# ParBLiSS/FastANI

Measured on AMD Instinct MI355X. Metric: ANI pairs/sec, many-to-many NxN ~5 Mbp genomes, higher is better.
Workload: dtype u32

## Files before the change

fastani_amd/csrc/engine_core.hip:

```cpp
#include "host/engine.hpp"
#include "kernels/scan.hpp"
#include "kernels/synth.hpp"

namespace anih {

thread_local std::string g_err;

int fail(int code, const char *fmt, ...)
{
  char buf[1024];
  va_list ap; va_start(ap, fmt); vsnprintf(buf, sizeof buf, fmt, ap); va_end(ap);
  g_err = buf;
  return code;
}

DevicePool g_pools[64];

int zero_counters(ani_ctx *c)
{
  HIP_TRY(hipMemsetAsync(c->dCounters.p, 0, kCounterWords * 8, c->stream));
  return ANI_OK;
}
int zero_cursors(ani_ctx *c, int pool)
{
// ... 133 lines not shown
  if (const char *ev = getenv("ANI_TEST_L2_OVERLAP")) c->l2Overlap = strcmp(ev, "0") != 0;
  if (const char *ev = getenv("ANI_TEST_L1_HIT_LIMIT")) { const long long v = atoll(ev);
    if (v >= 1) c->l1HitLimit = std::min<uint64_t>((uint64_t)v, 0x7ffffff0ull); }
  if (const char *ev = getenv("ANI_TEST_CAND_POOL_MIN")) { const long long v = atoll(ev); if (v >= 1) c->candPoolMin = (uint64_t)v; }
  if (const char *ev = getenv("ANI_TEST_L1_BIG_GROUP_HITS")) { const long long v = atoll(ev); if (v >= 1) c->l1BigGroupHits = (uint64_t)v; }
  if (const char *ev = getenv("ANI_TEST_L1_BIG_GROUP_FRAGS")) { const long long v = atoll(ev); if (v >= 1) c->l1BigGroupFrags = (uint64_t)v; }
  if (const char *ev = getenv("ANI_MAX_RESIDENT_CHUNKS")) { const long long v = atoll(ev);
    if (v >= 0) c->maxResidentChunks = (int32_t)std::min<long long>(v, 1 << 20); }
  if (const char *ev = getenv("ANI_STREAM_CHUNK_MINIMIZERS")) { const long long v = atoll(ev); if (v >= 1) c->streamChunkMinimizers = (uint64_t)v; }
  for (int i = 0; i < 2; i++) { HIP_TRY(hipEventCreateWithFlags(&c->evSimA[i], hipEventDisableTiming));
    HIP_TRY(hipEventCreateWithFlags(&c->evSetDone[i], hipEventDisableTiming)); HIP_TRY(hipEventCreateWithFlags(&c->evIndex[i], hipEventDisableTiming)); }
  int rc = c->dCounters.ensure(kCounterWords * 8);
  if (rc != ANI_OK) { delete c; return rc; }
  *out = c;
  return ANI_OK;
}

void ani_shutdown(ani_ctx *c)
{
  if (!c) return;
  (void)hipSetDevice(c->device);
  DevBuf *bufs[] = {&c->dCounters, &c->seqPacked, &c->seqAscii, &c->contigOff, &c->contigLen, &c->contigMode, &c->sortTmp, &c->unitStart, &c->unitAux,
      &c->tiles, &c->tileInfo, &c->tileMeta, &c->tileCnt,
                    &c->tileDrop, &c->tileOff, &c->poolHash, &c->poolWpos, &c->scanTmpA, &c->scanTmpB, &c->scanTmpC, &c->scanTmpD, &c->frags, &c->fragOff,
                        &c->fragS,
                    &c->fragGenome, &c->fragQSeq, &c->qPool, &c->l1FragDesc, &c->probeFirst, &c->probeCnt, &c->l1MidList, &c->l1SmallList, &c->l1BigList,
                        &c->l1BigHitsA, &c->l1BigHitsB, &c->l1BigV, &c->l1BigTbl, &c->l1BigHash, &c->candFrag, &c->candSeq, &c->candStart, &c->candEnd,
                        &c->fragCandOff, &c->fragCandCnt,
                    &c->fragCandCntClamped, &c->fragHits, &c->fragOrdOff, &c->fragOrder, &c->fragOrderTmp, &c->ocFrag, &c->ocSeq, &c->ocStart, &c->ocEnd,
                        &c->l2Scratch, &c->l2Ranges[0], &c->l2CodeCount[0], &c->l2CodeOff[0], &c->l2Codes[0], &c->l2SlowFlag[0], &c->l2ClassList[0],
                        &c->l2Order[0], &c->l2LenHist[0],
                    &c->l2Ranges[1], &c->l2CodeCount[1], &c->l2CodeOff[1], &c->l2Codes[1], &c->l2SlowFlag[1], &c->l2ClassList[1], &c->l2Order[1],
                        &c->l2LenHist[1], &c->l2SlowList, &c->l2Best,
                    &c->l2First, &c->l2Last, &c->refStart, &c->idBits, &c->keepFlags, &c->keepOff, &c->mapOut, &c->bins, &c->queryFragments, &c->rows};
  for (DevBuf *b : bufs) b->release();
  for (hipEvent_t e : c->timerEvents) if (e) (void)hipEventDestroy(e);
  for (int i = 0; i < 2; i++) { if (c->evSimA[i]) (void)hipEventDestroy(c->evSimA[i]); if (c->evSetDone[i]) (void)hipEventDestroy(c->evSetDone[i]);
    if (c->evIndex[i]) (void)hipEventDestroy(c->evIndex[i]); }
  if (c->stream2) (void)hipStreamDestroy(c->stream2);
  for (int i = 0; i < 5; i++) if (c->pinned[i]) (void)hipHostFree(c->pinned[i]);
  if (c->stream) (void)hipStreamDestroy(c->stream);
  delete c;
  cur_pool().trim();
}

int ani_device_copy(ani_ctx *c, void *dst, const void *src, size_t bytes)
{
  if (!c || (bytes && (!dst || !src))) return fail(ANI_ERR_ARG, "null argument");
  HIP_TRY(hipSetDevice(c->device));
  if (bytes) { HIP_TRY(hipMemcpyAsync(dst, src, bytes, hipMemcpyDefault, c->stream)); HIP_TRY(hipStreamSynchronize(c->stream)); }
  return ANI_OK;
}

int ani_device_alloc(ani_ctx *c, size_t bytes, void **out)
{
  if (!c || !out) return fail(ANI_ERR_ARG, "null argument");
  HIP_TRY(hipSetDevice(c->device));
  HIP_TRY(pool_malloc(out, bytes ? bytes : 1));
  return ANI_OK;
}

int ani_device_memory(ani_ctx *c, size_t *freeBytes, size_t *totalBytes)
{
  if (!c) return fail(ANI_ERR_ARG, "null argument");
  HIP_TRY(hipSetDevice(c->device));
  size_t f = 0, t = 0;
  HIP_TRY(hipMemGetInfo(&f, &t));
// ... 81 lines not shown
```

fastani_amd/csrc/engine_map.hip:

```cpp
#include <atomic>
#include <thread>
#include "host/engine.hpp"
#include "kernels/l1.hpp"
#include "kernels/l2.hpp"
#include "kernels/reduce.hpp"
#include "kernels/cluster.hpp"
#include "kernels/tree.hpp"
#include "kernels/nj.hpp"
#include "kernels/single.hpp"
#include "kernels/sigdist.hpp"
#include "kernels/sigstrip.hpp"
#include "kernels/signeigh.hpp"
#include "kernels/sigscreen.hpp"
#include "kernels/sigcontain.hpp"
#include "kernels/sigcluster.hpp"
#include "kernels/siggraph.hpp"

namespace anih {
using namespace ani;

void launch_l2_codes(unsigned grid, hipStream_t s, const L2FastArgs &fa);
void launch_l2_sim_a(unsigned grid, hipStream_t s, const L2FastArgs &fa, const int32_t *list, const unsigned int *listCount);
void launch_l2_sim_b(unsigned grid, hipStream_t s, const L2FastArgs &fa, const int32_t *list, const unsigned int *listCount);
static_assert(kL1FilterMinHits == 300 && kL1HitCapMax == 4080, "defaults of ani_ctx::l1FilterMin / l1LdsMax (host/engine.hpp)");
// ... 315 lines not shown
    if (nSlowTotal) {
      size_t lanes = (std::min<size_t>(nSlowTotal, (size_t)1 << 17) + kTPB - 1) / kTPB * kTPB;
      const size_t wordsPerLane = (size_t)maxS + 1;
      while (lanes > kTPB && lanes * wordsPerLane * 4 > ((size_t)2 << 30)) lanes = (lanes / 2 + kTPB - 1) / kTPB * kTPB;
      TRY(ctx->l2Scratch.ensure(lanes * wordsPerLane * 4));
      L2Args sa = a; sa.scratch = ctx->l2Scratch.as<uint32_t>(); sa.laneStride = lanes;
      StageTimer tk(ctx, &ctx->counters.msL2Slow, 1);
      for (size_t base = 0; base < nSlowTotal; base += lanes)
        hipLaunchKernelGGL(k_l2, dim3((unsigned)(lanes / kTPB)), dim3(kTPB), 0, ctx->stream, sa, (const int32_t *)ctx->l2SlowList.as<int32_t>(),
            (int32_t)nSlowTotal, (int32_t)base);
      HIP_TRY(hipGetLastError());
    }
    ctx->counters.l2SlowCandidates += nSlowTotal; ctx->counters.l2FastCandidates += nCand - nSlowTotal;
    FinishArgs fa;
    fa.nCand = (int32_t)nCand; fa.candFrag = a.candFrag; fa.candSeq = a.candSeq; fa.best = a.outBest; fa.firstPos = a.outFirst; fa.lastPos = a.outLast;
    fa.fragS = a.fragS; fa.idLUT = set->dIdLUT; fa.minShared = set->dMinShared; fa.lutMaxS = set->dLutMaxS;
    fa.refStart = ctx->refStart.as<int32_t>(); fa.idBits = ctx->idBits.as<uint32_t>();
    hipLaunchKernelGGL(k_finish_candidates, dim3(grid_for(nCand)), dim3(256), 0, ctx->stream, fa);
    HIP_TRY(hipGetLastError());
  }
  TRY(read_counters(ctx, host));
  ctx->counters.l2WindowEntries += host[CNT_ENTRIES] + host[CNT_ENTRIES_B]; ctx->counters.l2Steps += host[CNT_STEPS] + host[CNT_STEPS_B];
  ctx->counters.l2QueryHashes += host[CNT_SUMQ] + host[CNT_SUMQ_B];
  ctx->counters.l2WindowEntriesB += host[CNT_ENTRIES_B]; ctx->counters.l2QueryHashesB += host[CNT_SUMQ_B];
  ctx->counters.l2SlowLimit += host[CNT_REASON + 1]; ctx->counters.l2SlowDup += host[CNT_REASON + 2]; ctx->counters.l2SlowOverflow += host[CNT_REASON + 3];
  return ANI_OK;
}

int reduce_stage(ani_ctx *ctx, ani_sketch *set, IndexChunk *sk, const FragSet &fs, int32_t nCand, int32_t nQuery, bool compact = false)
{
  if (nQuery == 0 || sk->nGenomes == 0) return ANI_OK;
  const size_t binsPerQuery = sk->totalBins;
  const size_t nBins = binsPerQuery * (size_t)nQuery;
  TRY(ctx->bins.ensure((nBins ? nBins : 1) * 4));
  const size_t nPairsAll = (size_t)nQuery * (size_t)(compact ? sk->nGenomes : set->nGenomes);
  TRY(ctx->rows.ensure((nPairsAll ? nPairsAll : 1) * 8));
  hipError_t e1;
  {
  StageTimer tm(ctx, &ctx->counters.msReduce);
  e1 = hipMemsetAsync(ctx->bins.p, 0, (nBins ? nBins : 1) * 4, ctx->stream);
  if (nCand) {
    OneWayArgs a;
    a.nCand = nCand; a.candFrag = ctx->ocFrag.as<int32_t>(); a.candSeq = ctx->ocSeq.as<int32_t>(); a.refStart = ctx->refStart.as<int32_t>();
    a.idBits = ctx->idBits.as<uint32_t>(); a.fragGenome = fs.fragGenome; a.genomeBase = fs.genomeBase; a.contigGenome = sk->contigGenome;
    a.contigBinBase = sk->contigBinBase; a.binWidth = set->params.fragLen - 20; a.bins = ctx->bins.as<uint32_t>(); a.binsPerQuery = binsPerQuery;
    hipLaunchKernelGGL(k_oneway_bins, dim3(grid_for((size_t)nCand)), dim3(256), 0, ctx->stream, a);
  }
  PairArgs pa;
  pa.nQuery = nQuery; pa.nRefGenomes = sk->nGenomes; pa.bins = ctx->bins.as<uint32_t>(); pa.binsPerQuery = binsPerQuery;
  pa.genomeBinStart = sk->genomeBinStart; pa.pairCount = ctx->rows.as<uint32_t>(); pa.pairIdentity = ctx->rows.as<uint32_t>() + nPairsAll;
  pa.outStride = compact ? sk->nGenomes : set->nGenomes; pa.outCol0 = compact ? 0 : sk->g0;
  const size_t nPairs = (size_t)nQuery * (size_t)sk->nGenomes;
  hipLaunchKernelGGL(k_pair_reduce, dim3((unsigned)((nPairs + 3) / 4)), dim3(256), 0, ctx->stream, pa);
  }
  HIP_TRY(e1); HIP_TRY(hipGetLastError());
  return ANI_OK;
}

int collect_rows(ani_ctx *ctx, ani_sketch *set, const FragSet &fs, int32_t nQuery, int32_t firstQueryId, RowBuf *rows, const IndexChunk *block = nullptr,
    const int32_t *queryIds = nullptr)
{
  const int32_t nCols = block ? block->nGenomes : set->nGenomes, col0 = (block ? block->g0 : 0) + set->refIdBase;
  const size_t nPairs = (size_t)nQuery * (size_t)nCols;
  if (nPairs == 0) return ANI_OK;
  uint32_t *dense = nullptr;
  TRY(pinned_buffer(ctx, 1, nPairs * 8 + 8, (void **)&dense));
  HIP_TRY(hipMemcpyAsync(dense, ctx->rows.p, nPairs * 8, hipMemcpyDeviceToHost, ctx->stream));
  HIP_TRY(hipStreamSynchronize(ctx->stream));
  std::vector<size_t> qOff((size_t)nQuery + 1, 0);
  parallel_for((size_t)nQuery, (uint64_t)nPairs * 8, [&](size_t qi) {
    const uint32_t *cnt = dense + qi * (size_t)nCols;
    size_t c = 0;
    for (int32_t g = 0; g < nCols; g++) c += cnt[g] != 0;
    qOff[qi + 1] = c;
  });
  for (int32_t qi = 0; qi < nQuery; qi++) qOff[qi + 1] += qOff[qi];
  const size_t m = qOff[nQuery];
  ani_cgi_t *out0 = rows->grow(m);
  if (!out0) return fail(ANI_ERR_NOMEM, "host allocation of %zu result rows failed", m);
  rows->n += m;
  parallel_for((size_t)nQuery, (uint64_t)nPairs * 8, [&](size_t qi) {
    const uint32_t *cnt = dense + qi * (size_t)nCols, *idb = cnt + nPairs;
    ani_cgi_t *out = out0 + qOff[qi];
    for (int32_t g = 0; g < nCols; g++) {
      if (!cnt[g]) continue;
      ani_cgi_t r; r.refGenomeId = col0 + g; r.qryGenomeId = firstQueryId + (queryIds ? queryIds[qi] : (int32_t)qi); r.countSeq = (int32_t)cnt[g];
      r.totalQueryFragments = fs.genomeFragments[qi];
      memcpy(&r.identity, &idb[g], 4);
// ... 1747 lines not shown
```

fastani_amd/csrc/engine_sketch.hip:

```cpp
#include "host/engine.hpp"
#include "kernels/reduce.hpp"
#include "kernels/sketch.hpp"

namespace anih {
using namespace ani;

int check_params(const ani_params_t *p)
{
  if (!p) return fail(ANI_ERR_ARG, "null parameters");
  if (p->kmerSize < 1 || p->kmerSize > 16) return fail(ANI_ERR_ARG, "kmerSize must be in 1..16 (hash_t is 32 bit, parseCmdArgs.hpp:142)");
  if (p->windowSize < 1 || p->windowSize > ani::kTile - ani::kTPB) return fail(ANI_ERR_LIMIT, "windowSize %d outside 1..%d", p->windowSize,
      ani::kTile - ani::kTPB);
  if (p->fragLen < 1 || p->fragLen <= 20) return fail(ANI_ERR_ARG, "fragLen must exceed 20 (bin width is fragLen-20, computeCoreIdentity.hpp:194)");
  return ANI_OK;
}

int frag_tables(ani_ctx *ctx, const ani_params_t &p, const DeviceBatch &db, FragSet *qr, std::vector<uint32_t> *fragStartOut, const FragArrays &fa, bool alloc,
                FragArrays *owned)
{
  const int k = p.kmerSize, w = p.windowSize, L = p.fragLen;
  std::vector<uint32_t> &fragStart = *fragStartOut;
  fragStart.assign((size_t)db.nContigs + 1, 0);
  std::vector<int32_t> cGenome((size_t)db.nContigs + 1, 0), cQBase((size_t)db.nContigs + 1, 0);
  qr->genomeFragments.assign(db.nGenomes, 0);
// ... 123 lines not shown
    TRY(ctx->poolHash.ensure(cap * 4)); TRY(ctx->poolWpos.ensure(cap * 4));
    if (fused && (!*fused->qPool || attempt > 0)) {
      if (*fused->qPool) { pool_free(*fused->qPool); *fused->qPool = nullptr; }
      HIP_TRY(pool_malloc((void **)fused->qPool, (qcap ? qcap : 1) * 4));
    }
    TRY(zero_counters(ctx));
    {
      StageTimer tm(ctx, &ctx->counters.msSketch);
      if (!fused)
        hipLaunchKernelGGL(k_sketch_tiles, dim3((unsigned)nT), dim3(kTPB), 0, ctx->stream, db.dPacked, db.dAscii, db.dContigOff,
                           db.dContigLen, db.dContigMode, ctx->tiles.as<TileDesc>(), k, w, ctx->poolHash.as<uint32_t>(),
                           ctx->poolWpos.as<int32_t>(), stripe_cap(cap), cur_ptr(ctx, POOL_REF), ctx->tileMeta.as<TileMeta>());
      else
        hipLaunchKernelGGL(k_sketch_fused, dim3((unsigned)nT), dim3(kTPB), 0, ctx->stream, db.dPacked, db.dAscii, db.dContigOff, db.dContigLen, db.dContigMode,
                           ctx->tiles.as<TileDesc>(), ctx->tileInfo.as<FusedInfo>(), k, w, L, ctx->poolHash.as<uint32_t>(), ctx->poolWpos.as<int32_t>(),
                               stripe_cap(cap),
                           cur_ptr(ctx, POOL_REF), ctx->tileMeta.as<TileMeta>(), *fused->qPool, stripe_cap(qcap), cur_ptr(ctx,
                               POOL_Q), fused->arr->fragOff, fused->arr->fragS,
                           (int *)cnt_ptr(ctx, CNT_MAXS));
    }
    HIP_TRY(hipGetLastError());
    TRY(read_counters(ctx, host));
    const bool refFits = ctx->poolMaxStripe[POOL_REF] <= stripe_cap(cap), qFits = !fused || ctx->poolMaxStripe[POOL_Q] <= stripe_cap(qcap);
    if (refFits && qFits) break;
    if (attempt > 2) return fail(ANI_ERR_INTERNAL, "minimizer pool did not converge");
    if (!refFits) cap = grown_cap(ctx->poolMaxStripe[POOL_REF]);
    if (!qFits) qcap = grown_cap(ctx->poolMaxStripe[POOL_Q]);
  }
  if (fused) {
    const int maxS = (int)(uint32_t)host[CNT_MAXS];
    if (maxS >= 0x7fffffff) return fail(ANI_ERR_LIMIT, "a query fragment produced more than %d minimizers", kFragHashCap);
    const uint64_t nHashes = ctx->poolUsed[POOL_Q];
    ctx->counters.querySketchHashes += nHashes;
    uint32_t *packed = nullptr;
    TRY(compact_fragment_pool(ctx, *fused->qPool, fused->arr->fragOff, fused->arr->fragS, nF, nHashes, &packed));
    pool_free(*fused->qPool); *fused->qPool = packed;
    fused->fs->maxS = maxS; fused->fs->nHashes = nHashes; fused->fs->poolSize = nHashes; fused->fs->qPool = *fused->qPool;
  }
  StageTimer tm(ctx, &ctx->counters.msSketch);
  hipLaunchKernelGGL(k_sketch_tile_counts, dim3(grid_for(nT)), dim3(256), 0, ctx->stream, ctx->tiles.as<TileDesc>(),
                     ctx->tileMeta.as<TileMeta>(), (int)nT, ctx->tileCnt.as<int32_t>(), ctx->tileDrop.as<uint8_t>());
  uint64_t total = 0;
  TRY(device_scan(ctx, ctx->tileCnt.as<int32_t>(), ctx->tileOff.as<uint32_t>(), (uint32_t)nT, &total));
  if (total >= 0x7ffffff0ull) return fail(ANI_ERR_LIMIT, "reference batch yields >= 2^31 minimizers; split the reference list");
  if (total == 0) return ANI_OK;
  uint32_t *rec = nullptr;
  HIP_TRY(pool_malloc((void **)&rec, total * 12));
  hipLaunchKernelGGL(k_sketch_gather, dim3((unsigned)nT), dim3(kTPB), 0, ctx->stream, ctx->tiles.as<TileDesc>(), ctx->tileMeta.as<TileMeta>(),
                     ctx->tileDrop.as<uint8_t>(), ctx->tileOff.as<uint32_t>(), ctx->poolHash.as<uint32_t>(), ctx->poolWpos.as<int32_t>(),
                     seqIdBase, rec);
  hipError_t e = hipGetLastError();
  if (e == hipSuccess) e = hipStreamSynchronize(ctx->stream);
  if (e != hipSuccess) { pool_free(rec); HIP_TRY(e); }
  *dRecords = rec; *nOut = (size_t)total;
  return ANI_OK;
}

int fragment_stage(ani_ctx *ctx, const ani_params_t &p, const DeviceBatch &db, FragSet *qr)
{
  if (ctx->timerPending.size() > 4096) flush_timers(ctx);
  const int k = p.kmerSize, w = p.windowSize, L = p.fragLen;
  {
    uint64_t nF = 0;
    for (int32_t c = 0; c < db.nContigs; c++) { const int32_t len = db.contigLen[c]; if (!(len < w || len < k || len < L)) nF += (uint64_t)(len / L); }
    TRY(ctx->fragOff.ensure((nF + 1) * 4)); TRY(ctx->fragS.ensure((nF + 1) * 4)); TRY(ctx->fragGenome.ensure((nF + 1) * 4));
    TRY(ctx->fragQSeq.ensure((nF + 1) * 4));
  }
  FragArrays fa; fa.fragOff = ctx->fragOff.as<uint32_t>(); fa.fragS = ctx->fragS.as<int32_t>(); fa.fragGenome = ctx->fragGenome.as<int32_t>();
  fa.fragQSeq = ctx->fragQSeq.as<int32_t>();
  std::vector<uint32_t> fragStart;
// ... 32 lines not shown
  qr->qPool = ctx->qPool.as<uint32_t>();
  return ANI_OK;
}

void fragset_release(ani_fragset *f)
{
  void *tables[] = {f->arr.fragOff, f->arr.fragS, f->arr.fragGenome, f->arr.fragQSeq};
  if (!f->borrowed || f->ownTables) for (void *q : tables) if (q) pool_free(q);
  if (!f->borrowed && f->qPool) pool_free(f->qPool);
  delete f;
}
void fragset_finish(ani_fragset *f)
{
  f->genomeFragStart.assign(f->fs.genomeFragments.size() + 1, 0);
  for (size_t g = 0; g < f->fs.genomeFragments.size(); g++) f->genomeFragStart[g + 1] = f->genomeFragStart[g] + f->fs.genomeFragments[g];
}
int keep_fragment_arrays(ani_ctx *ctx, ani_fragset *f)
{
  const size_t nF = (size_t)f->fs.nFrag;
  if (!nF) return ANI_OK;
  hipError_t e = pool_malloc((void **)&f->arr.fragOff, nF * 4); if (e == hipSuccess) e = pool_malloc((void **)&f->arr.fragS, nF * 4);
  if (e == hipSuccess) e = pool_malloc((void **)&f->arr.fragGenome, nF * 4); if (e == hipSuccess) e = pool_malloc((void **)&f->arr.fragQSeq, nF * 4);
  if (e == hipSuccess) e = hipMemcpyAsync(f->arr.fragOff, f->fs.fragOff, nF * 4, hipMemcpyDeviceToDevice, ctx->stream);
  if (e == hipSuccess) e = hipMemcpyAsync(f->arr.fragS, f->fs.fragS, nF * 4, hipMemcpyDeviceToDevice, ctx->stream);
  if (e == hipSuccess) e = hipMemcpyAsync(f->arr.fragGenome, f->fs.fragGenome, nF * 4, hipMemcpyDeviceToDevice, ctx->stream);
  if (e == hipSuccess) e = hipMemcpyAsync(f->arr.fragQSeq, f->fs.fragQSeq, nF * 4, hipMemcpyDeviceToDevice, ctx->stream);
  if (e != hipSuccess) return fail(e == hipErrorOutOfMemory ? ANI_ERR_NOMEM : ANI_ERR_DEVICE, "keeping the fragment sketches failed: %s", hipGetErrorString(e));
  TRY(compact_fragment_pool(ctx, f->fs.qPool, f->arr.fragOff, f->arr.fragS, nF, f->fs.nHashes, &f->qPool));
  f->fs.fragOff = f->arr.fragOff; f->fs.fragS = f->arr.fragS; f->fs.fragGenome = f->arr.fragGenome; f->fs.fragQSeq = f->arr.fragQSeq;
  f->fs.qPool = f->qPool; f->fs.poolSize = f->fs.nHashes;
  return ANI_OK;
}

int records_of_batch(ani_ctx *ctx, const ani_params_t *p, const ani_seq_batch_t *refs, int32_t seqIdBase, void **devRecords, size_t *n, ani_fragset *keep)
{
  std::vector<RecordPart> parts;
  auto cleanup = [&]() { for (auto &q : parts) if (q.rec) pool_free(q.rec); };
  size_t total = 0;
  int32_t g0 = 0;
  while (g0 < refs->nGenomes) {
    int32_t g1 = g0; uint64_t bases = 0;
    while (g1 < refs->nGenomes && (g1 == g0 || keep || bases < (1ull << 30))) {
      for (int32_t c = refs->genomeContigStart[g1]; c < refs->genomeContigStart[g1 + 1]; c++) bases += (uint64_t)refs->contigLen[c];
      g1++;
    }
    DeviceBatch db;
    int rc = upload_batch(ctx, refs, g0, g1, &db);
    RecordPart pt; pt.g0 = g0; pt.g1 = g1;
    if (rc == ANI_OK) {
      if (keep && fusable(p)) {
        FusedOut fo{&keep->fs, &keep->arr, &keep->qPool};
        rc = sketch_records(ctx, p, db, seqIdBase + refs->genomeContigStart[g0], &pt.rec, &pt.n, &fo);
      } else {
        rc = sketch_records(ctx, p, db, seqIdBase + refs->genomeContigStart[g0], &pt.rec, &pt.n);
        if (rc == ANI_OK && keep) {
          rc = fragment_stage(ctx, *p, db, &keep->fs);
          if (rc == ANI_OK) rc = keep_fragment_arrays(ctx, keep);
        }
      }
    }
    if (rc != ANI_OK) { cleanup(); return rc; }
    parts.push_back(pt); total += pt.n;
    g0 = g1;
  }
  uint32_t *all = nullptr;
  if (parts.size() == 1) { all = parts[0].rec; parts[0].rec = nullptr; }
  else if (total) {
    hipError_t e = pool_malloc((void **)&all, total * 12);
    size_t o = 0;
    for (size_t i = 0; i < parts.size() && e == hipSuccess; i++) {
      if (parts[i].n) e = hipMemcpyAsync(all + 3 * o, parts[i].rec, parts[i].n * 12, hipMemcpyDeviceToDevice, ctx->stream);
      o += parts[i].n;
    }
    if (e == hipSuccess) e = hipStreamSynchronize(ctx->stream);
    if (e != hipSuccess) { if (all) pool_free(all); cleanup();
      return fail(e == hipErrorOutOfMemory ? ANI_ERR_NOMEM : ANI_ERR_DEVICE, "gathering %zu records failed: %s", total, hipGetErrorString(e)); }
  }
  cleanup();
  if (ctx->timerPending.size() > 1024) flush_timers(ctx);
  *devRecords = all; *n = total;
  return ANI_OK;
}

}
// ... 30 lines not shown
  HIP_TRY(hipSetDevice(ctx->device));
  ani_fragset *f = new ani_fragset();
  f->ctx = ctx; f->device = ctx->device; f->params = *p;
  DeviceBatch db;
  int rc = upload_batch(ctx, queries, 0, queries->nGenomes, &db);
  if (rc == ANI_OK) rc = fragment_stage(ctx, *p, db, &f->fs);
  if (rc == ANI_OK) rc = keep_fragment_arrays(ctx, f);
  if (rc != ANI_OK) { fragset_release(f); return rc; }
  fragset_finish(f);
  *out = f;
  return ANI_OK;
}

void ani_fragset_free(ani_fragset *f)
{
  if (!f) return;
  (void)hipSetDevice(f->device);
  fragset_release(f);
}

namespace {
struct FragWireHeader {
  char magic[8]; uint32_t version; int32_t kmerSize, windowSize, fragLen; float percentageIdentity;
  int32_t nFrag, nGenomes, maxS; uint64_t nHashes, poolSize;
  uint64_t offGenomeFragments, offFragOff, offFragS, offFragGenome, offFragQSeq, offPool, totalBytes;
};
static_assert(sizeof(FragWireHeader) <= 256, "wire header fits its slot");
inline uint64_t wire_align(uint64_t x) { return (x + 255) / 256 * 256; }
FragWireHeader wire_header(const ani_fragset *f)
{
  FragWireHeader h; memset(&h, 0, sizeof h);
  memcpy(h.magic, "ANIFRAGS", 8); h.version = 1;
  h.kmerSize = f->params.kmerSize; h.windowSize = f->params.windowSize; h.fragLen = f->params.fragLen; h.percentageIdentity = f->params.percentageIdentity;
  h.nFrag = f->fs.nFrag; h.nGenomes = (int32_t)f->fs.genomeFragments.size(); h.maxS = f->fs.maxS; h.nHashes = f->fs.nHashes; h.poolSize = f->fs.poolSize;
  const uint64_t nF = (uint64_t)h.nFrag;
  h.offGenomeFragments = 256;
  h.offFragOff = wire_align(h.offGenomeFragments + (uint64_t)h.nGenomes * 4);
  h.offFragS = wire_align(h.offFragOff + nF * 4);
  h.offFragGenome = wire_align(h.offFragS + nF * 4);
  h.offFragQSeq = wire_align(h.offFragGenome + nF * 4);
  h.offPool = wire_align(h.offFragQSeq + nF * 4);
  h.totalBytes = wire_align(h.offPool + h.poolSize * 4);
  return h;
}
const char *validate_wire_header(const FragWireHeader &h, uint64_t bytesAvailable)
{
  if (memcmp(h.magic, "ANIFRAGS", 8) != 0 || h.version != 1) return "not a packed fragment set";
  if (h.nFrag < 0 || h.nGenomes < 0 || h.maxS < 0 || h.poolSize > 0xfffffff0ull || h.nHashes > h.poolSize) return "inconsistent counts";
  ani_fragset tmp; tmp.fs.nFrag = h.nFrag; tmp.fs.poolSize = h.poolSize; tmp.fs.genomeFragments.assign((size_t)h.nGenomes, 0);
  const FragWireHeader want = wire_header(&tmp);
  if (want.offGenomeFragments != h.offGenomeFragments || want.offFragOff != h.offFragOff || want.offFragS != h.offFragS
      || want.offFragGenome != h.offFragGenome ||
      want.offFragQSeq != h.offFragQSeq || want.offPool != h.offPool || want.totalBytes != h.totalBytes || h.totalBytes > bytesAvailable)
    return "truncated or malformed";
  return nullptr;
}
}

int ani_fragset_pack_bytes(const ani_fragset *f, size_t *bytes)
{
  if (!f || !bytes) return fail(ANI_ERR_ARG, "null argument");
  *bytes = (size_t)wire_header(f).totalBytes;
  return ANI_OK;
}

int ani_fragset_pack(ani_ctx *ctx, const ani_fragset *f, void *devBuf, size_t cap, size_t *bytes)
{
  if (!ctx || !f || !devBuf) return fail(ANI_ERR_ARG, "null argument");
  if (f->device != ctx->device) return fail(ANI_ERR_ARG, "fragment set lives on device %d, context on %d", f->device, ctx->device);
  HIP_TRY(hipSetDevice(ctx->device));
  const FragWireHeader h = wire_header(f);
  if (h.totalBytes > cap) return fail(ANI_ERR_ARG, "buffer of %zu bytes is too small for a fragment set of %llu bytes", cap, (unsigned long long)h.totalBytes);
  uint8_t *b = (uint8_t *)devBuf;
  const size_t nF = (size_t)h.nFrag;
  HIP_TRY(hipMemcpyAsync(b, &h, sizeof h, hipMemcpyHostToDevice, ctx->stream));
  if (h.nGenomes) HIP_TRY(hipMemcpyAsync(b + h.offGenomeFragments, f->fs.genomeFragments.data(), (size_t)h.nGenomes * 4, hipMemcpyHostToDevice, ctx->stream));
  if (nF) {
    HIP_TRY(hipMemcpyAsync(b + h.offFragOff, f->fs.fragOff, nF * 4, hipMemcpyDeviceToDevice, ctx->stream));
    HIP_TRY(hipMemcpyAsync(b + h.offFragS, f->fs.fragS, nF * 4, hipMemcpyDeviceToDevice, ctx->stream));
    HIP_TRY(hipMemcpyAsync(b + h.offFragGenome, f->fs.fragGenome, nF * 4, hipMemcpyDeviceToDevice, ctx->stream));
    HIP_TRY(hipMemcpyAsync(b + h.offFragQSeq, f->fs.fragQSeq, nF * 4, hipMemcpyDeviceToDevice, ctx->stream));
  }
  if (h.poolSize) HIP_TRY(hipMemcpyAsync(b + h.offPool, f->fs.qPool, (size_t)h.poolSize * 4, hipMemcpyDeviceToDevice, ctx->stream));
  HIP_TRY(hipStreamSynchronize(ctx->stream));
  if (bytes) *bytes = (size_t)h.totalBytes;
  return ANI_OK;
}

int ani_fragset_unpack(ani_ctx *ctx, const void *devBuf, size_t bytes, ani_fragset **out)
{
  if (!ctx || !devBuf || !out) return fail(ANI_ERR_ARG, "null argument");
  HIP_TRY(hipSetDevice(ctx->device));
  if (bytes < 256) return fail(ANI_ERR_ARG, "not a packed fragment set");
  FragWireHeader h;
  HIP_TRY(hipMemcpy(&h, devBuf, sizeof h, hipMemcpyDeviceToHost));
  if (const char *why = validate_wire_header(h, bytes)) return fail(ANI_ERR_ARG, "packed fragment set: %s", why);
  ani_fragset tmp; tmp.params.kmerSize = h.kmerSize; tmp.params.windowSize = h.windowSize; tmp.params.fragLen = h.fragLen;
  tmp.params.percentageIdentity = h.percentageIdentity;
  TRY(check_params(&tmp.params));
  tmp.fs.nFrag = h.nFrag; tmp.fs.maxS = h.maxS; tmp.fs.nHashes = h.nHashes; tmp.fs.poolSize = h.poolSize; tmp.fs.genomeFragments.assign((size_t)h.nGenomes, 0);
  ani_fragset *f = new ani_fragset();
  f->ctx = ctx; f->device = ctx->device; f->params = tmp.params; f->borrowed = true;
  f->fs = tmp.fs;
// ... 131 lines not shown
```

fastani_amd/csrc/host/engine.hpp:

```cpp
#pragma once
#include <hip/hip_runtime.h>

#include <fcntl.h>
#include <sys/mman.h>
#include <sys/stat.h>
#include <unistd.h>

#include <algorithm>
#include <array>
#include <atomic>
#include <thread>
#include <chrono>
#include <condition_variable>
#include <functional>
#include <memory>
#include <cstdarg>
#include <cstdint>
#include <cstdio>
#include <cstdlib>
#include <cstring>
#include <map>
#include <mutex>
#include <set>
#include <string>
// ... 295 lines not shown
  bool l1Tiny = true;
  bool l2Overlap = true;
  uint64_t l1HitLimit = 0x7ffffff0ull;
  uint64_t candPoolMin = 4096;
  uint64_t l1BigGroupHits = 1ull << 27, l1BigGroupFrags = 1ull << 20;
  int32_t maxResidentChunks = 0;
  uint64_t streamChunkMinimizers = 1000000000ull;
  std::vector<std::unique_ptr<ani::stat::Luts>> lutCache;
  void *pinned[5] = {nullptr, nullptr, nullptr, nullptr, nullptr}; size_t pinnedCap[5] = {0, 0, 0, 0, 0};
  hipStream_t stream2 = nullptr;
  hipEvent_t evSimA[2] = {nullptr, nullptr}, evSetDone[2] = {nullptr, nullptr}, evIndex[2] = {nullptr, nullptr};
  std::vector<hipEvent_t> timerEvents; size_t timerUsed = 0;
  struct PendingTimer { size_t a, b; double *acc; };
  std::vector<PendingTimer> timerPending;
  ani_counters_t counters;
  std::vector<unsigned long long> hostCounters;
  unsigned long long poolUsed[3] = {0, 0, 0}, poolMaxStripe[3] = {0, 0, 0};
  double candPerFrag = 12.0;
  double candSeen[32] = {0}; int candSeenAt = 0;
  uint64_t smallBatchCandCap = 0;
  DevBuf dCounters;
  DevBuf seqPacked, seqAscii, contigOff, contigLen, contigMode;
  DevBuf sortTmp, unitStart, unitAux, tiles, tileInfo, tileMeta, tileCnt, tileDrop, tileOff, poolHash, poolWpos;
  DevBuf scanTmpA, scanTmpB, scanTmpC, scanTmpD;
  DevBuf frags, fragOff, fragS, fragGenome, fragQSeq, qPool;
  DevBuf l1FragDesc;
  DevBuf probeFirst, probeCnt, l1MidList, l1SmallList, l1BigList, l1BigHitsA, l1BigHitsB, l1BigV, l1BigTbl, l1BigHash, candFrag, candSeq, candStart, candEnd,
      fragCandOff, fragCandCnt, fragCandCntClamped, fragHits, fragOrdOff, fragOrder, fragOrderTmp;
  DevBuf ocFrag, ocSeq, ocStart, ocEnd;
  DevBuf l2Scratch, l2Best, l2First, l2Last, refStart, idBits, keepFlags, keepOff, mapOut;
  DevBuf l2Ranges[2], l2CodeCount[2], l2CodeOff[2], l2Codes[2], l2SlowFlag[2], l2ClassList[2], l2Order[2], l2LenHist[2];
  DevBuf l2SlowList;
  DevBuf bins, queryFragments, rows;
};

struct RecordPiece { const uint32_t *rec; size_t n; };
struct IndexChunk {
  uint32_t n = 0;
  int32_t c0 = 0, nContigs = 0, g0 = 0, nGenomes = 0;
  uint64_t nUnique = 0;
  bool resident = false, everBuilt = false;
  uint64_t lastUse = 0;
  std::vector<RecordPiece> pieces;
  uint32_t *mHash = nullptr; int32_t *mSeq = nullptr, *mWpos = nullptr;
  uint32_t *sHash = nullptr, *mWin = nullptr;
  uint32_t *dupBits = nullptr; uint64_t *dupList = nullptr; uint32_t nDup = 0;
  uint64_t *sSW = nullptr;
  ani::TableSlot *table = nullptr; uint32_t tableSlots = 0;
  int32_t *contigFirstMin = nullptr, *contigGenome = nullptr;
  uint32_t *contigBinBase = nullptr, *genomeBinStart = nullptr, *posBase = nullptr, *posSample = nullptr;
  uint32_t totalBins = 0, totalPosBins = 0;
  int32_t maxContigLen = 0;
};

struct ani_sketch {
  ani_ctx *ctx = nullptr;
  int device = 0;
  ani_params_t params;
  uint64_t n = 0;
  int32_t nContigs = 0, nGenomes = 0;
  uint64_t totalLen = 0;
  int32_t refIdBase = 0;
  uint64_t nUnique = 0; bool uniqueExact = false;
  std::vector<int32_t> contigLen, genomeContigStart;
  std::vector<std::string> genomeNames;
  std::vector<IndexChunk *> chunks;
// ... 50 lines not shown
struct DeviceBatch {
  int32_t nGenomes = 0, nContigs = 0;
  std::vector<int32_t> genomeContigStart, contigLen;
  std::vector<int64_t> contigOff;
  std::vector<uint8_t> contigPacked;
  const uint32_t *dPacked = nullptr; const uint8_t *dAscii = nullptr;
  const int64_t *dContigOff = nullptr; const int32_t *dContigLen = nullptr; const uint8_t *dContigMode = nullptr;
  uint64_t totalBases = 0;
};
int check_batch(const ani_seq_batch_t *b);
int check_params(const ani_params_t *p);
}

struct ani_dev_batch {
  ani_ctx *ctx = nullptr; int device = 0;
  DeviceBatch db;
  void *bufs[5] = {nullptr, nullptr, nullptr, nullptr, nullptr};
};
struct ani_fragset;

namespace anih {
int upload_batch(ani_ctx *ctx, const ani_seq_batch_t *b, int32_t g0, int32_t g1, DeviceBatch *out, ani_dev_batch *keep = nullptr);

struct FragSet {
  int32_t nFrag = 0, maxS = 0;
  uint64_t nHashes = 0;
  uint64_t poolSize = 0;
  std::vector<int32_t> genomeFragments;
  const uint32_t *qPool = nullptr, *fragOff = nullptr; const int32_t *fragS = nullptr, *fragGenome = nullptr, *fragQSeq = nullptr;
  int32_t genomeBase = 0;
};

struct FragArrays { uint32_t *fragOff = nullptr; int32_t *fragS = nullptr, *fragGenome = nullptr, *fragQSeq = nullptr; };
struct FusedOut { FragSet *fs; FragArrays *arr; uint32_t **qPool; };
struct RecordPart { uint32_t *rec = nullptr; size_t n = 0; int32_t g0 = 0, g1 = 0; bool owned = true; };
struct RowBuf {
  ani_cgi_t *p = nullptr; size_t n = 0, cap = 0;
  ani_cgi_t *grow(size_t extra)
  {
    if (n + extra > cap || !p) {
      size_t want = std::max<size_t>(n + extra, cap + cap / 2 + 1024);
      void *q = realloc(p, want * sizeof(ani_cgi_t));
      if (!q) return nullptr;
      p = (ani_cgi_t *)q; cap = want;
    }
    return p + n;
  }
  ~RowBuf() { free(p); }
  ani_cgi_t *release() { ani_cgi_t *r = p ? p : (ani_cgi_t *)malloc(sizeof(ani_cgi_t)); p = nullptr; return r; }
};

}

struct ani_fragset {
  ani_ctx *ctx = nullptr; int device = 0;
  ani_params_t params;
  FragSet fs;
  FragArrays arr; uint32_t *qPool = nullptr;
  bool borrowed = false;
  std::vector<int64_t> genomeFragStart;
  std::vector<int32_t> genomeQueryId;
  bool ownTables = false;
};


namespace anih {
int sketch_records(ani_ctx *ctx, const ani_params_t *p, const DeviceBatch &db, int32_t seqIdBase, uint32_t **dRecords, size_t *nOut, FusedOut *fused = nullptr);
int fragment_stage(ani_ctx *ctx, const ani_params_t &p, const DeviceBatch &db, FragSet *qr);
void free_chunk_index(IndexChunk *ch);
void free_chunk(IndexChunk *ch);
void free_sketch_device(ani_sketch *sk);
int upload_luts(ani_sketch *sk, int maxS);
ani_sketch *new_sketch(ani_ctx *ctx, const ani_params_t *p, const int32_t *contigLen, int32_t nContigs, const int32_t *genomeContigStart, int32_t nGenomes);
int ensure_chunk(ani_sketch *sk, size_t i, int pin = -1);
int add_chunks(ani_ctx *ctx, ani_sketch *sk, std::vector<RecordPart> &parts);
int exact_unique(ani_sketch *sk);

template <class T> int to_host_malloc(const std::vector<T> &v, T **out, size_t *n)
{
  *n = v.size();
  *out = (T *)malloc((v.size() ? v.size() : 1) * sizeof(T));
  if (!*out) return fail(ANI_ERR_NOMEM, "host allocation failed");
  if (!v.empty()) memcpy(*out, v.data(), v.size() * sizeof(T));
  return ANI_OK;
}
}
```

fastani_amd/csrc/kernels/reduce.hpp:

```cpp
#pragma once
#include "common.hpp"

namespace ani {

__host__ __device__ __forceinline__ uint32_t lut_off(int s) { return (uint32_t)(((int64_t)(s - 1) * (s + 2)) / 2); }

struct FinishArgs {
  int32_t nCand;
  const int32_t *candFrag, *candSeq;
  const int32_t *best, *firstPos, *lastPos;
  const int32_t *fragS;
  const uint32_t *idLUT; const int32_t *minShared; int32_t lutMaxS;
  int32_t *refStart;
  uint32_t *idBits;
};

static __global__ void k_finish_candidates(FinishArgs a)
{
  const int c = blockIdx.x * blockDim.x + threadIdx.x;
  if (c >= a.nCand) return;
  const int s = a.fragS[a.candFrag[c]];
  const int b = a.best[c];
  a.refStart[c] = (a.firstPos[c] + a.lastPos[c]) / 2;
  uint32_t bits = 0;
  if (b > 0 && s <= a.lutMaxS && b >= a.minShared[s]) bits = a.idLUT[lut_off(s) + b];
  a.idBits[c] = bits;
}

struct OneWayArgs {
  int32_t nCand;
  const int32_t *candFrag, *candSeq, *refStart; const uint32_t *idBits;
  const int32_t *fragGenome;
  int32_t genomeBase;
  const int32_t *contigGenome;
  const uint32_t *contigBinBase;
  int32_t binWidth;
  uint32_t *bins; size_t binsPerQuery;
};

static __global__ void k_oneway_bins(OneWayArgs a)
{
  const int c = blockIdx.x * blockDim.x + threadIdx.x;
  if (c >= a.nCand) return;
  const int f = a.candFrag[c];
  const int g = a.contigGenome[a.candSeq[c]];
  if (c > 0 && a.candFrag[c - 1] == f && a.contigGenome[a.candSeq[c - 1]] == g) return;
  uint32_t bBits = 0; int32_t bSeq = -1, bPos = -1;
  for (int x = c; x < a.nCand && a.candFrag[x] == f && a.contigGenome[a.candSeq[x]] == g; x++) {
    const uint32_t bits = a.idBits[x];
    if (!bits) continue;
    const int32_t sq = a.candSeq[x], ps = a.refStart[x];
    if (bits > bBits || (bits == bBits && (sq > bSeq || (sq == bSeq && ps > bPos)))) { bBits = bits; bSeq = sq; bPos = ps; }
  }
  if (bBits) {
    const size_t bin = (size_t)(a.fragGenome[f] - a.genomeBase) * a.binsPerQuery + a.contigBinBase[bSeq] + (uint32_t)(bPos / a.binWidth);
    atomicMax(&a.bins[bin], bBits);
  }
}

struct PairArgs {
  int32_t nQuery, nRefGenomes;
  const uint32_t *bins; size_t binsPerQuery;
  const uint32_t *genomeBinStart;
  uint32_t *pairCount; uint32_t *pairIdentity; int32_t outStride, outCol0;
};

static __global__ __launch_bounds__(kTPB) void k_pair_reduce(PairArgs a)
{
  const long long p = ((long long)blockIdx.x * kTPB + threadIdx.x) >> 6;
  if (p >= (long long)a.nQuery * a.nRefGenomes) return;
  const int lane = threadIdx.x & (kWave - 1);
  const int qi = (int)(p / a.nRefGenomes), g = (int)(p % a.nRefGenomes);
  const uint32_t *b = a.bins + (size_t)qi * a.binsPerQuery;
  const uint32_t x1 = a.genomeBinStart[g + 1];
  float sum = 0.0f; int cnt = 0;
  for (uint32_t x0 = a.genomeBinStart[g]; x0 < x1; x0 += kWave) {
    const uint32_t bits = (x0 + lane < x1) ? b[x0 + lane] : 0u;
    unsigned long long m = __ballot(bits != 0);
    cnt += __popcll(m);
    while (m) {
      const int l = __ffsll(m) - 1;
      sum += __uint_as_float((uint32_t)__builtin_amdgcn_readlane((int)bits, l));
      m &= m - 1;
    }
  }
  if (lane == 0) {
    const size_t o = (size_t)qi * (size_t)a.outStride + (size_t)(a.outCol0 + g);
    a.pairCount[o] = (uint32_t)cnt;
    a.pairIdentity[o] = cnt ? __float_as_uint(sum / cnt) : 0u;
  }
}

static __global__ void k_emit_mappings(int32_t nCand, const int32_t *__restrict__ candFrag, const int32_t *__restrict__ candSeq,
                                const int32_t *__restrict__ refStart, const uint32_t *__restrict__ idBits,
                                const int32_t *__restrict__ best, const int32_t *__restrict__ fragS,
                                const int32_t *__restrict__ fragQuerySeqId, const uint32_t *__restrict__ outOff, int L,
                                int32_t seqBase ,
                                uint32_t *__restrict__ out )
{
  const int c = blockIdx.x * blockDim.x + threadIdx.x;
  if (c >= nCand || !idBits[c]) return;
  uint32_t *m = out + 11 * (size_t)outOff[c];
  const int f = candFrag[c];
  m[0] = (uint32_t)L; m[1] = (uint32_t)refStart[c]; m[2] = (uint32_t)(refStart[c] + L - 1); m[3] = 0; m[4] = (uint32_t)(L - 1);
  m[5] = (uint32_t)(candSeq[c] + seqBase); m[6] = (uint32_t)fragQuerySeqId[f]; m[7] = idBits[c]; m[8] = 0;
  m[9] = (uint32_t)fragS[f]; m[10] = (uint32_t)best[c];
}

static __global__ void k_keep_flags(int32_t n, const uint32_t *__restrict__ idBits, int32_t *__restrict__ flags)
{
  const int c = blockIdx.x * blockDim.x + threadIdx.x;
  if (c < n) flags[c] = idBits[c] != 0;
}

static __global__ void k_clamp_counts(int32_t n, const int32_t *__restrict__ in, const int32_t *__restrict__ order, int32_t *__restrict__ out)
{
  const int i = blockIdx.x * blockDim.x + threadIdx.x;
// ... 13 lines not shown
```

Before: 5.242 million.

## Track occupied bin slabs to skip empty bins and avoid per-call bin clearing

Adds a per-pair occupancy bitmask, set by the one-way binning kernel, so the pair reduction only scans bin slabs that received hits. The reduction zeroes the bins and masks it reads, so the full memset of the bin buffer runs only when the buffer is reallocated or a previous call left it dirty. Separately, query fragment pool compaction is deferred from sketching to the point where the fragment set is serialized, so the fused path keeps the striped pool. Together these cut memset bandwidth and sparse bin scanning at the cost of extra atomics and added state-tracking complexity.

```diff
diff --git a/fastani_amd/csrc/engine_core.hip b/fastani_amd/csrc/engine_core.hip
--- a/fastani_amd/csrc/engine_core.hip
+++ b/fastani_amd/csrc/engine_core.hip
@@ -189,7 +189,7 @@
                         &c->l2Order[0], &c->l2LenHist[0],
                     &c->l2Ranges[1], &c->l2CodeCount[1], &c->l2CodeOff[1], &c->l2Codes[1], &c->l2SlowFlag[1], &c->l2ClassList[1], &c->l2Order[1],
                         &c->l2LenHist[1], &c->l2SlowList, &c->l2Best,
-                    &c->l2First, &c->l2Last, &c->refStart, &c->idBits, &c->keepFlags, &c->keepOff, &c->mapOut, &c->bins, &c->queryFragments, &c->rows};
+                    &c->l2First, &c->l2Last, &c->refStart, &c->idBits, &c->keepFlags, &c->keepOff, &c->mapOut, &c->bins, &c->binOcc, &c->queryFragments, &c->rows};
   for (DevBuf *b : bufs) b->release();
   for (hipEvent_t e : c->timerEvents) if (e) (void)hipEventDestroy(e);
   for (int i = 0; i < 2; i++) { if (c->evSimA[i]) (void)hipEventDestroy(c->evSimA[i]); if (c->evSetDone[i]) (void)hipEventDestroy(c->evSetDone[i]);
diff --git a/fastani_amd/csrc/engine_map.hip b/fastani_amd/csrc/engine_map.hip
--- a/fastani_amd/csrc/engine_map.hip
+++ b/fastani_amd/csrc/engine_map.hip
@@ -371,28 +371,35 @@
   if (nQuery == 0 || sk->nGenomes == 0) return ANI_OK;
   const size_t binsPerQuery = sk->totalBins;
   const size_t nBins = binsPerQuery * (size_t)nQuery;
+  const size_t nPairs = (size_t)nQuery * (size_t)sk->nGenomes;
+  const size_t capBins = ctx->bins.cap, capOcc = ctx->binOcc.cap;
+  const bool wasDirty = ctx->binsDirty;
+  ctx->binsDirty = true;
   TRY(ctx->bins.ensure((nBins ? nBins : 1) * 4));
+  TRY(ctx->binOcc.ensure(nPairs * 4));
+  const bool clearBins = wasDirty || ctx->bins.cap != capBins, clearOcc = wasDirty || ctx->binOcc.cap != capOcc;
   const size_t nPairsAll = (size_t)nQuery * (size_t)(compact ? sk->nGenomes : set->nGenomes);
   TRY(ctx->rows.ensure((nPairsAll ? nPairsAll : 1) * 8));
-  hipError_t e1;
   {
   StageTimer tm(ctx, &ctx->counters.msReduce);
-  e1 = hipMemsetAsync(ctx->bins.p, 0, (nBins ? nBins : 1) * 4, ctx->stream);
+  if (clearBins) HIP_TRY(hipMemsetAsync(ctx->bins.p, 0, ctx->bins.cap, ctx->stream));
+  if (clearOcc) HIP_TRY(hipMemsetAsync(ctx->binOcc.p, 0, ctx->binOcc.cap, ctx->stream));
   if (nCand) {
     OneWayArgs a;
     a.nCand = nCand; a.candFrag = ctx->ocFrag.as<int32_t>(); a.candSeq = ctx->ocSeq.as<int32_t>(); a.refStart = ctx->refStart.as<int32_t>();
     a.idBits = ctx->idBits.as<uint32_t>(); a.fragGenome = fs.fragGenome; a.genomeBase = fs.genomeBase; a.contigGenome = sk->contigGenome;
     a.contigBinBase = sk->contigBinBase; a.binWidth = set->params.fragLen - 20; a.bins = ctx->bins.as<uint32_t>(); a.binsPerQuery = binsPerQuery;
+    a.genomeBinStart = sk->genomeBinStart; a.occ = ctx->binOcc.as<uint32_t>(); a.nRefGenomes = sk->nGenomes;
     hipLaunchKernelGGL(k_oneway_bins, dim3(grid_for((size_t)nCand)), dim3(256), 0, ctx->stream, a);
   }
   PairArgs pa;
-  pa.nQuery = nQuery; pa.nRefGenomes = sk->nGenomes; pa.bins = ctx->bins.as<uint32_t>(); pa.binsPerQuery = binsPerQuery;
+  pa.nQuery = nQuery; pa.nRefGenomes = sk->nGenomes; pa.bins = ctx->bins.as<uint32_t>(); pa.binsPerQuery = binsPerQuery; pa.occ = ctx->binOcc.as<uint32_t>();
   pa.genomeBinStart = sk->genomeBinStart; pa.pairCount = ctx->rows.as<uint32_t>(); pa.pairIdentity = ctx->rows.as<uint32_t>() + nPairsAll;
   pa.outStride = compact ? sk->nGenomes : set->nGenomes; pa.outCol0 = compact ? 0 : sk->g0;
-  const size_t nPairs = (size_t)nQuery * (size_t)sk->nGenomes;
   hipLaunchKernelGGL(k_pair_reduce, dim3((unsigned)((nPairs + 3) / 4)), dim3(256), 0, ctx->stream, pa);
   }
-  HIP_TRY(e1); HIP_TRY(hipGetLastError());
+  HIP_TRY(hipGetLastError());
+  ctx->binsDirty = false;
   return ANI_OK;
 }
 
diff --git a/fastani_amd/csrc/engine_sketch.hip b/fastani_amd/csrc/engine_sketch.hip
--- a/fastani_amd/csrc/engine_sketch.hip
+++ b/fastani_amd/csrc/engine_sketch.hip
@@ -179,10 +179,8 @@
     if (maxS >= 0x7fffffff) return fail(ANI_ERR_LIMIT, "a query fragment produced more than %d minimizers", kFragHashCap);
     const uint64_t nHashes = ctx->poolUsed[POOL_Q];
     ctx->counters.querySketchHashes += nHashes;
-    uint32_t *packed = nullptr;
-    TRY(compact_fragment_pool(ctx, *fused->qPool, fused->arr->fragOff, fused->arr->fragS, nF, nHashes, &packed));
-    pool_free(*fused->qPool); *fused->qPool = packed;
-    fused->fs->maxS = maxS; fused->fs->nHashes = nHashes; fused->fs->poolSize = nHashes; fused->fs->qPool = *fused->qPool;
+    fused->fs->maxS = maxS; fused->fs->nHashes = nHashes; fused->fs->poolSize = qcap; fused->fs->qPool = *fused->qPool;
+    *fused->striped = true;
   }
   StageTimer tm(ctx, &ctx->counters.msSketch);
   hipLaunchKernelGGL(k_sketch_tile_counts, dim3(grid_for(nT)), dim3(256), 0, ctx->stream, ctx->tiles.as<TileDesc>(),
@@ -281,6 +279,25 @@
   return ANI_OK;
 }
 
+int fragset_packed(ani_ctx *ctx, const ani_fragset *fc)
+{
+  if (!fc->striped) return ANI_OK;
+  ani_fragset *f = const_cast<ani_fragset *>(fc);
+  const size_t nF = (size_t)f->fs.nFrag;
+  uint32_t *off = nullptr, *packed = nullptr;
+  if (nF) {
+    HIP_TRY(pool_malloc((void **)&off, nF * 4));
+    const hipError_t e = hipMemcpyAsync(off, f->arr.fragOff, nF * 4, hipMemcpyDeviceToDevice, ctx->stream);
+    if (e != hipSuccess) { pool_free(off); HIP_TRY(e); }
+  }
+  const int rc = compact_fragment_pool(ctx, f->qPool, off, f->arr.fragS, nF, f->fs.nHashes, &packed);
+  if (rc != ANI_OK) { pool_free(off); return rc; }
+  pool_free(f->qPool); f->qPool = packed;
+  if (nF) { pool_free(f->arr.fragOff); f->arr.fragOff = off; f->fs.fragOff = off; }
+  f->fs.qPool = packed; f->fs.poolSize = f->fs.nHashes; f->striped = false;
+  return ANI_OK;
+}
+
 int records_of_batch(ani_ctx *ctx, const ani_params_t *p, const ani_seq_batch_t *refs, int32_t seqIdBase, void **devRecords, size_t *n, ani_fragset *keep)
 {
   std::vector<RecordPart> parts;
@@ -298,7 +315,7 @@
     RecordPart pt; pt.g0 = g0; pt.g1 = g1;
     if (rc == ANI_OK) {
       if (keep && fusable(p)) {
-        FusedOut fo{&keep->fs, &keep->arr, &keep->qPool};
+        FusedOut fo{&keep->fs, &keep->arr, &keep->qPool, &keep->striped};
         rc = sketch_records(ctx, p, db, seqIdBase + refs->genomeContigStart[g0], &pt.rec, &pt.n, &fo);
       } else {
         rc = sketch_records(ctx, p, db, seqIdBase + refs->genomeContigStart[g0], &pt.rec, &pt.n);
@@ -395,7 +412,8 @@
   FragWireHeader h; memset(&h, 0, sizeof h);
   memcpy(h.magic, "ANIFRAGS", 8); h.version = 1;
   h.kmerSize = f->params.kmerSize; h.windowSize = f->params.windowSize; h.fragLen = f->params.fragLen; h.percentageIdentity = f->params.percentageIdentity;
-  h.nFrag = f->fs.nFrag; h.nGenomes = (int32_t)f->fs.genomeFragments.size(); h.maxS = f->fs.maxS; h.nHashes = f->fs.nHashes; h.poolSize = f->fs.poolSize;
+  h.nFrag = f->fs.nFrag; h.nGenomes = (int32_t)f->fs.genomeFragments.size(); h.maxS = f->fs.maxS; h.nHashes = f->fs.nHashes;
+  h.poolSize = f->striped ? f->fs.nHashes : f->fs.poolSize;
   const uint64_t nF = (uint64_t)h.nFrag;
   h.offGenomeFragments = 256;
   h.offFragOff = wire_align(h.offGenomeFragments + (uint64_t)h.nGenomes * 4);
@@ -432,6 +450,7 @@
   if (!ctx || !f || !devBuf) return fail(ANI_ERR_ARG, "null argument");
   if (f->device != ctx->device) return fail(ANI_ERR_ARG, "fragment set lives on device %d, context on %d", f->device, ctx->device);
   HIP_TRY(hipSetDevice(ctx->device));
+  TRY(fragset_packed(ctx, f));
   const FragWireHeader h = wire_header(f);
   if (h.totalBytes > cap) return fail(ANI_ERR_ARG, "buffer of %zu bytes is too small for a fragment set of %llu bytes", cap, (unsigned long long)h.totalBytes);
   uint8_t *b = (uint8_t *)devBuf;
diff --git a/fastani_amd/csrc/host/engine.hpp b/fastani_amd/csrc/host/engine.hpp
--- a/fastani_amd/csrc/host/engine.hpp
+++ b/fastani_amd/csrc/host/engine.hpp
@@ -351,6 +351,7 @@
   DevBuf l2Ranges[2], l2CodeCount[2], l2CodeOff[2], l2Codes[2], l2SlowFlag[2], l2ClassList[2], l2Order[2], l2LenHist[2];
   DevBuf l2SlowList;
   DevBuf bins, queryFragments, rows;
+  DevBuf binOcc; bool binsDirty = false;
 };
 
 struct RecordPiece { const uint32_t *rec; size_t n; };
@@ -467,7 +468,7 @@
 };
 
 struct FragArrays { uint32_t *fragOff = nullptr; int32_t *fragS = nullptr, *fragGenome = nullptr, *fragQSeq = nullptr; };
-struct FusedOut { FragSet *fs; FragArrays *arr; uint32_t **qPool; };
+struct FusedOut { FragSet *fs; FragArrays *arr; uint32_t **qPool; bool *striped; };
 struct RecordPart { uint32_t *rec = nullptr; size_t n = 0; int32_t g0 = 0, g1 = 0; bool owned = true; };
 struct RowBuf {
   ani_cgi_t *p = nullptr; size_t n = 0, cap = 0;
@@ -492,6 +493,7 @@
   ani_params_t params;
   FragSet fs;
   FragArrays arr; uint32_t *qPool = nullptr;
+  bool striped = false;
   bool borrowed = false;
   std::vector<int64_t> genomeFragStart;
   std::vector<int32_t> genomeQueryId;
diff --git a/fastani_amd/csrc/kernels/reduce.hpp b/fastani_amd/csrc/kernels/reduce.hpp
--- a/fastani_amd/csrc/kernels/reduce.hpp
+++ b/fastani_amd/csrc/kernels/reduce.hpp
@@ -36,7 +36,11 @@
   const uint32_t *contigBinBase;
   int32_t binWidth;
   uint32_t *bins; size_t binsPerQuery;
+  const uint32_t *genomeBinStart;
+  uint32_t *occ; int32_t nRefGenomes;
 };
+
+__host__ __device__ __forceinline__ uint32_t occ_slab(uint32_t nBins) { return nBins > 2048u ? 64u * ((nBins + 2047u) / 2048u) : 64u; }
 
 static __global__ void k_oneway_bins(OneWayArgs a)
 {
@@ -53,14 +57,17 @@
     if (bits > bBits || (bits == bBits && (sq > bSeq || (sq == bSeq && ps > bPos)))) { bBits = bits; bSeq = sq; bPos = ps; }
   }
   if (bBits) {
-    const size_t bin = (size_t)(a.fragGenome[f] - a.genomeBase) * a.binsPerQuery + a.contigBinBase[bSeq] + (uint32_t)(bPos / a.binWidth);
-    atomicMax(&a.bins[bin], bBits);
+    const size_t q = (size_t)(a.fragGenome[f] - a.genomeBase);
+    const uint32_t bin = a.contigBinBase[bSeq] + (uint32_t)(bPos / a.binWidth), x0 = a.genomeBinStart[g];
+    atomicMax(&a.bins[q * a.binsPerQuery + bin], bBits);
+    atomicOr(&a.occ[q * (size_t)a.nRefGenomes + (size_t)g], 1u << ((bin - x0) / occ_slab(a.genomeBinStart[g + 1] - x0)));
   }
 }
 
 struct PairArgs {
   int32_t nQuery, nRefGenomes;
-  const uint32_t *bins; size_t binsPerQuery;
+  uint32_t *bins; size_t binsPerQuery;
+  uint32_t *occ;
   const uint32_t *genomeBinStart;
   uint32_t *pairCount; uint32_t *pairIdentity; int32_t outStride, outCol0;
 };
@@ -71,18 +78,26 @@
   if (p >= (long long)a.nQuery * a.nRefGenomes) return;
   const int lane = threadIdx.x & (kWave - 1);
   const int qi = (int)(p / a.nRefGenomes), g = (int)(p % a.nRefGenomes);
-  const uint32_t *b = a.bins + (size_t)qi * a.binsPerQuery;
-  const uint32_t x1 = a.genomeBinStart[g + 1];
+  uint32_t occ = (uint32_t)__builtin_amdgcn_readlane((int)a.occ[p], 0);
   float sum = 0.0f; int cnt = 0;
-  for (uint32_t x0 = a.genomeBinStart[g]; x0 < x1; x0 += kWave) {
-    const uint32_t bits = (x0 + lane < x1) ? b[x0 + lane] : 0u;
-    unsigned long long m = __ballot(bits != 0);
-    cnt += __popcll(m);
-    while (m) {
-      const int l = __ffsll(m) - 1;
-      sum += __uint_as_float((uint32_t)__builtin_amdgcn_readlane((int)bits, l));
-      m &= m - 1;
+  if (occ) {
+    uint32_t *b = a.bins + (size_t)qi * a.binsPerQuery;
+    const uint32_t g0 = a.genomeBinStart[g], x1 = a.genomeBinStart[g + 1], S = occ_slab(x1 - g0);
+    for (; occ; occ &= occ - 1) {
+      const uint32_t s0 = g0 + (uint32_t)(__ffs(occ) - 1) * S, s1 = (x1 - s0 > S) ? s0 + S : x1;
+      for (uint32_t x0 = s0; x0 < s1; x0 += kWave) {
+        const uint32_t bits = (x0 + lane < s1) ? b[x0 + lane] : 0u;
+        unsigned long long m = __ballot(bits != 0);
+        if (bits) b[x0 + lane] = 0u;
+        cnt += __popcll(m);
+        while (m) {
+          const int l = __ffsll(m) - 1;
+          sum += __uint_as_float((uint32_t)__builtin_amdgcn_readlane((int)bits, l));
+          m &= m - 1;
+        }
+      }
     }
+    if (lane == 0) a.occ[p] = 0u;
   }
   if (lane == 0) {
     const size_t o = (size_t)qi * (size_t)a.outStride + (size_t)(a.outCol0 + g);
```

Measured after the change: 5.329 million (median of 6 runs). 1.7% higher.
